# barbararoessle/e2e_multi_view_matching

Measured on AMD Instinct MI355X. Metric: image-pairs/sec @1024 kpts + pose AUC@5/10/20deg vs reference, higher is better.
Workload: dtype f16x2 (fp32 operands carried as 2 fp16 planes hi + 2^-11 lo', 22 significant bits, 3 fp16-MFMA products, fp32 accumulate; same 1e-4 / bit-exact-index parity bar); 1 GPU; configs[1]: tuple_size=2 (1 pair per tuple), 1024 keypoints, 256-dim f32 descriptors, GNN 9x1 = 18 layers, 100 Sinkhorn iters, batch 32 tuples/GPU = 32 pairs/GPU, w8pt pose per pair; pairs_per_gpu=32, global_pairs=32, weights=random init (timed), identity-like for the AUC leg, parallelism=tuple-sharded x1

## Files before the change

e2e_multi_view_matching_amd/csrc/attention_p2w.hip:

```cpp
#include <algorithm>
#include <type_traits>

#include "attention_p2.h"

namespace e2emv {

typedef __attribute__((ext_vector_type(16))) float aw_f32x16;

constexpr int AW_QT = 256;
constexpr int AW_TILEB = 64 * 256;
constexpr int AW_REGB = 2 * AW_TILEB;
constexpr int AW_ELS = 3 * AW_REGB;
constexpr int AW_QIMG = AW_ELS + 2048;
constexpr int AW_LDS = AW_QIMG + 3 * AW_TILEB;
constexpr int AW_PART_F = 68;
constexpr float AW_SINV = 1.f / P2_QS, AW_PLOG = 7.f, AW_LIMIT = 60000.f;

__device__ __forceinline__ void aw_wait_q_k0(p2_f16x8 (&q)[2][2][4]) {
    asm volatile("s_waitcnt vmcnt(0) lgkmcnt(0)\n\ts_barrier"
                 : "+a"(q[0][0][0]), "+a"(q[0][0][1]), "+a"(q[0][0][2]), "+a"(q[0][0][3]), "+a"(q[0][1][0]), "+a"(q[0][1][1]), "+a"(q[0][1][2]), "+a"(q[0][1][3]),
                   "+a"(q[1][0][0]), "+a"(q[1][0][1]), "+a"(q[1][0][2]), "+a"(q[1][0][3]), "+a"(q[1][1][0]), "+a"(q[1][1][1]), "+a"(q[1][1][2]), "+a"(q[1][1][3])
                 :: "memory");
}

template <int I, int N, class F>
__device__ __forceinline__ void aw_for(F&& f) {
    if constexpr (I < N) {
        f(std::integral_constant<int, I>{});
        aw_for<I + 1, N>(f);
    }
}

__device__ __forceinline__ unsigned aw_cvt_pk(float v0, float v1) {
    const p2_f32x2 vv = {v0, v1};
    return __builtin_bit_cast(unsigned, __builtin_convertvector(vv, p2_f16x2));
}
__device__ __forceinline__ float aw_fma(float a, float b, float c) {
    float d;
    asm volatile("v_fma_f32 %0, %1, %2, %3" : "=v"(d) : "v"(a), "v"(b), "v"(c));
    return d;
}
__device__ __forceinline__ float aw_exp2(float a) {
    float d;
    asm volatile("v_exp_f32 %0, %1" : "=v"(d) : "v"(a));
    return d;
}
__device__ __forceinline__ void aw_acc(float& sum, float a) { asm volatile("v_add_f32 %0, %0, %1" : "+v"(sum) : "v"(a)); }
__device__ __forceinline__ unsigned aw_cvt_pk_v(float v0, float v1) {
    unsigned d;
    asm volatile("v_cvt_pk_f16_f32 %0, %1, %2" : "=v"(d) : "v"(v0), "v"(v1));
    return d;
}
__device__ __forceinline__ unsigned aw_mixlo(unsigned hi, float v0) {
    unsigned lo;
    asm volatile("v_fma_mixlo_f16 %0, %1, -1.0, %2 op_sel_hi:[1,0,0]" : "=v"(lo) : "v"(hi), "v"(v0));
    return lo;
}
__device__ __forceinline__ unsigned aw_mixhi(unsigned lo, unsigned hi, float v1) {
    asm volatile("v_fma_mixhi_f16 %0, %1, -1.0, %2 op_sel:[1,0,0] op_sel_hi:[1,0,0]" : "+v"(lo) : "v"(hi), "v"(v1));
    return lo;
}
__device__ __forceinline__ unsigned aw_lo(unsigned hi, float v0, float v1) {
    unsigned lo;
    asm("v_fma_mixlo_f16 %0, %1, -1.0, %2 op_sel_hi:[1,0,0]\n\tv_fma_mixhi_f16 %0, %1, -1.0, %3 op_sel:[1,0,0] op_sel_hi:[1,0,0]"
        : "=&v"(lo) : "v"(hi), "v"(v0), "v"(v1));
    return lo;
}

__device__ __forceinline__ void aw_mfma_s(aw_f32x16& c, p2_f16x8 a, p2_f16x8 b) {
    asm volatile("v_mfma_f32_32x32x16_f16 %0, %1, %2, %0" : "+v"(c) : "v"(a), "a"(b));
}
__device__ __forceinline__ void aw_mfma_s0(aw_f32x16& c, p2_f16x8 a, p2_f16x8 b) {
    asm volatile("v_mfma_f32_32x32x16_f16 %0, %1, %2, 0" : "=&v"(c) : "v"(a), "a"(b));
}
__device__ __forceinline__ void aw_mfma_sa(aw_f32x16& c, p2_f16x8 a, p2_f16x8 b) {
    asm volatile("v_mfma_f32_32x32x16_f16 %0, %1, %2, %0" : "+v"(c) : "a"(a), "a"(b));
}
__device__ __forceinline__ void aw_mfma_sa0(aw_f32x16& c, p2_f16x8 a, p2_f16x8 b) {
    asm volatile("v_mfma_f32_32x32x16_f16 %0, %1, %2, 0" : "=&v"(c) : "a"(a), "a"(b));
}
__device__ __forceinline__ void aw_mfma_oa(aw_f32x16& c, p2_f16x8 a, p2_u32x4 b) {
    asm volatile("v_mfma_f32_32x32x16_f16 %0, %1, %2, %0" : "+a"(c) : "a"(a), "v"(b));
}
template <int IMM>
__device__ __forceinline__ void aw_read_frag(p2_f16x8& d, unsigned addr) {
    static_assert(IMM >= 0 && IMM < 65536, "ds_read offset: 16 bits");
    asm volatile("ds_read_b128 %0, %1 offset:%2" : "=a"(d) : "v"(addr), "n"(IMM));
}
template <int N>
__device__ __forceinline__ void aw_wait_frag(p2_f16x8 (&f)[4]) {
    asm volatile("s_waitcnt lgkmcnt(%4)" : "+a"(f[0]), "+a"(f[1]), "+a"(f[2]), "+a"(f[3]) : "n"(N));
}
template <bool HAS_E, bool MULTI = true, bool PART = false>
__global__ __launch_bounds__(256, 1) void attention_p2w_kernel(AttnP2Params p) {
    extern __shared__ __attribute__((aligned(16))) char smem_aw[];

    int lin = blockIdx.x, ks = 0;
    constexpr bool part = PART;
    if constexpr (PART) {
        const int h = blockIdx.x, tpx = (8 * p.gper * p.nq - p.n_full) >> 3;
        ks = (h >> 3) / tpx;
        lin = p.n_full + 8 * ((h >> 3) % tpx) + (h & 7);
    }
    const int xcd = lin & 7, idx = lin >> 3;
    const int g = xcd * p.gper + idx / p.nq;
    if (g >= p.groups) return;
    const int qt = idx % p.nq;
    const int img = g / p.H, head = g % p.H;
    const int b = img / p.T, t = img % p.T;
    if (qt * AW_QT >= p.nv[t]) return;

    const int tid = threadIdx.x, lane = tid & 63;
    const int wave = __builtin_amdgcn_readfirstlane(tid >> 6);
    const int l31 = lane & 31, lh = lane >> 5;
    const unsigned row_b = 8u * (unsigned)p.D;

    int q_row[2];
    bool q_ok[2];
    p2_f16x8 Qf[2][2][4];
#pragma unroll
    for (int a = 0; a < 2; ++a) {
        q_row[a] = qt * AW_QT + wave * 64 + a * 32 + l31;
        q_ok[a] = q_row[a] < p.n_rows;
    }
    const int q_blk = __builtin_amdgcn_readfirstlane(((int64_t)img * p.n_rows + min(qt * AW_QT + wave * 64, p.n_rows - 1)) >> 6);
    const int e_q_v = HAS_E ? p.EQK[q_blk * 8 + head] : 0;
    const unsigned q_img = wave == 0 ? 2u * AW_REGB : (unsigned)(AW_QIMG + (wave - 1) * AW_TILEB);
    {
        const __amdgpu_buffer_rsrc_t rsQ = __builtin_amdgcn_make_buffer_rsrc(const_cast<uint16_t*>(p.qk), 0, (int)p.qk_bytes, 0x00020000);
        const unsigned so = (unsigned)(img * p.n_rows) * row_b;
        asm volatile("" ::: "memory");
#pragma unroll
        for (int i = 0; i < 16; ++i) {
            const int rl = 4 * i + (lane >> 4);
            const int row = min(qt * AW_QT + wave * 64 + rl, p.n_rows - 1);
            const unsigned c = (unsigned)((lane & 15) ^ (rl & 15));
            p2_glds16(rsQ, smem_aw + q_img + i * 1024, (unsigned)row * row_b + (unsigned)head * 256u + c * 16u, so);
        }
        asm volatile("" ::: "memory");
    }
    const int e_q = __builtin_amdgcn_readfirstlane(e_q_v);

    const int n_src = p.cross ? p.T - 1 : 1;
    auto src_t = [&](int si) __attribute__((always_inline)) { return !p.cross ? t : (si < t ? si : si + 1); };
    int n_tiles = 0;
    for (int si = 0; si < n_src; ++si) n_tiles += (p.nv[src_t(si)] + 63) / 64;
    int t0 = 0;
    if constexpr (PART) {
        t0 = ks * n_tiles / p.n_split;
        n_tiles = (ks + 1) * n_tiles / p.n_split - t0;
        if (n_tiles <= 0) return;
    }
    struct Cur { int si, kt, nv; unsigned kb, vb; int eb; };
    auto cur_src = [&](Cur& c) __attribute__((always_inline)) {
        const int im = b * p.T + src_t(c.si);
        c.kt = 0;
        c.nv = p.nv[src_t(c.si)];
        c.kb = (unsigned)(im * p.n_rows) * row_b;
        c.vb = (unsigned)((im * p.H + head) * 64) * (unsigned)p.n_rows * 4u;
        c.eb = (im * p.n_rows) >> 6;
    };
    auto cur_next = [&](Cur& c) __attribute__((always_inline)) {
        ++c.kt;
        if constexpr (MULTI) {
            if (c.kt * 64 >= c.nv && c.si + 1 < n_src) { ++c.si; cur_src(c); }
        }
    };
    auto cur_init = [&]() __attribute__((always_inline)) {
        Cur c;
        c.si = 0;
        cur_src(c);
        if constexpr (PART)
            for (int i = 0; i < t0; ++i) cur_next(c);
        return c;
    };

    const __amdgpu_buffer_rsrc_t rsK = __builtin_amdgcn_make_buffer_rsrc(const_cast<uint16_t*>(p.qk), 0, (int)p.qk_bytes, 0x00020000);
    const __amdgpu_buffer_rsrc_t rsV = __builtin_amdgcn_make_buffer_rsrc(const_cast<uint16_t*>(p.vt), 0, (int)p.vt_bytes, 0x00020000);
    unsigned k_vo[4], v_vo[4];
#pragma unroll
    for (int i = 0; i < 4; ++i) {
        const int row = 4 * (wave * 4 + i) + (lane >> 4);
        const unsigned c = (unsigned)((lane & 15) ^ (row & 15));
        k_vo[i] = (unsigned)row * row_b + 4u * (unsigned)p.D + (unsigned)head * 256u + c * 16u;
        v_vo[i] = (unsigned)row * (unsigned)p.n_rows * 4u + c * 16u;
    }
    auto k_so = [&](const Cur& c) __attribute__((always_inline)) { return c.kb + (unsigned)c.kt * 64u * row_b; };
    auto v_so = [&](const Cur& c) __attribute__((always_inline)) { return c.vb + (unsigned)c.kt * 256u; };
    auto k_piece = [&](int region, int i, unsigned so) __attribute__((always_inline)) { p2_glds16(rsK, smem_aw + region * AW_REGB + AW_TILEB + (wave * 4 + i) * 1024, k_vo[i], so); };
    auto v_piece = [&](int region, int i, unsigned so) __attribute__((always_inline)) { p2_glds16(rsV, smem_aw + region * AW_REGB + (wave * 4 + i) * 1024, v_vo[i], so); };
    int* const els = reinterpret_cast<int*>(smem_aw + AW_ELS);
    int ek_mine = 0, ev_mine = 0;
    if (HAS_E && tid < n_tiles) {
        int si = 0, kt = PART ? tid + t0 : tid;
        if constexpr (MULTI) {
            for (; si + 1 < n_src; ++si) {
                const int nt = (p.nv[src_t(si)] + 63) / 64;
                if (kt < nt) break;
                kt -= nt;
            }
        }
        const int blk = (((b * p.T + src_t(si)) * p.n_rows) >> 6) + kt;
        ek_mine = p.EQK[blk * 8 + 4 + head];
        if (p.EVt) ev_mine = p.EVt[blk * 4 + head];
    }
    typedef __attribute__((address_space(3))) const p2_u32x2* lds_pair_t;
    const unsigned els0 = (unsigned)(uintptr_t)(__attribute__((address_space(3))) char*)smem_aw + (unsigned)AW_ELS;
    auto read_e = [&](int tl) __attribute__((always_inline)) {
        return *reinterpret_cast<lds_pair_t>((uintptr_t)(els0 + 8u * (unsigned)min(tl, n_tiles - 1)));
    };

    const int kz = l31 & 15;
    const unsigned lds0 = (unsigned)(uintptr_t)(__attribute__((address_space(3))) char*)smem_aw;
    unsigned R[4][2];
#pragma unroll
    for (int s = 0; s < 4; ++s)
#pragma unroll
        for (int pl = 0; pl < 2; ++pl)
            R[s][pl] = lds0 + (unsigned)(l31 * 256 + ((((s >> 1) * 8 + pl * 4 + 2 * (s & 1) + lh) ^ kz) << 4));
    typedef __attribute__((address_space(3))) const p2_f16x8* lds_frag_t;
    auto frag = [&](int s, int pl, int imm) __attribute__((always_inline)) { return *reinterpret_cast<lds_frag_t>((uintptr_t)(R[s][pl] + (unsigned)imm)); };

    constexpr int PA[3] = {1, 0, 0};
    constexpr int PB[3] = {0, 1, 0};

    aw_f32x16 O[2][2], S[2][2];
    p2_u32x4 Pf[2][2][4];
#pragma unroll
    for (int a = 0; a < 2; ++a)
#pragma unroll
        for (int d = 0; d < 2; ++d)
#pragma unroll
            for (int r = 0; r < 16; ++r) O[a][d][r] = 0.f;
    float m_run[2] = {-1e30f, -1e30f}, l_run[2] = {0.f, 0.f};
    int e_o = 0;
    bool o_started = false;
    unsigned n_slow = 0;

    auto sm_slow = [&](auto BB, float sinv, int valid) __attribute__((always_inline)) {
        constexpr int B = decltype(BB)::value;
        asm volatile("s_nop 15" : "+v"(S[B][0]), "+v"(S[B][1]), "+a"(O[B][0]), "+a"(O[B][1]));
        if (valid < 64) {
#pragma unroll
            for (int kb = 0; kb < 2; ++kb)
#pragma unroll
                for (int r = 0; r < 16; ++r)
                    if (kb * 32 + (r & 3) + 8 * (r >> 2) + 4 * lh >= valid) S[B][kb][r] = -INFINITY;
        }
        float mx = S[B][0][0];
#pragma unroll
        for (int kb = 0; kb < 2; ++kb)
#pragma unroll
            for (int r = 0; r < 16; ++r) mx = fmaxf(mx, S[B][kb][r]);
        {
            float x = mx, y = mx;
            asm volatile("s_nop 1\n\tv_permlane32_swap_b32 %0, %1\n\ts_nop 1" : "+v"(x), "+v"(y));
            mx = fmaxf(x, y);
        }
        mx *= sinv;
        const float m_new = fmaxf(m_run[B], mx);
        const float alpha = __builtin_amdgcn_exp2f(m_run[B] - m_new);
#pragma unroll
        for (int r = 0; r < 16; ++r) { O[B][0][r] *= alpha; O[B][1][r] *= alpha; }
        const float e0 = AW_PLOG - m_new;
        float ps = 0.f;
#pragma unroll
        for (int k = 0; k < 16; ++k) {
            const int kb = k >> 3, r = 2 * (k & 7), u = 2 * kb + ((k & 7) >> 2), e = k & 3;
            const float p0 = __builtin_amdgcn_exp2f(__builtin_fmaf(S[B][kb][r], sinv, e0));
            const float p1 = __builtin_amdgcn_exp2f(__builtin_fmaf(S[B][kb][r + 1], sinv, e0));
            ps += p0 + p1;
            const P2Pair pr = p2_split_plain(p0, p1);
            Pf[B][0][u][e] = pr.hi; Pf[B][1][u][e] = pr.lo;
        }
        l_run[B] = l_run[B] * alpha + ps;
        m_run[B] = m_new;
        asm volatile("s_nop 4" : "+a"(O[B][0]), "+a"(O[B][1]));
    };

    Cur cK = cur_init(), cV = cur_init(), cS = cur_init();
    int nK = 0, nV = 0;
    auto adv_k = [&]() __attribute__((always_inline)) { if (++nK < n_tiles) cur_next(cK); };
    auto adv_v = [&]() __attribute__((always_inline)) { if (++nV < n_tiles) cur_next(cV); };
    {
        const unsigned so = k_so(cK);
#pragma unroll
        for (int i = 0; i < 4; ++i) k_piece(2, i, so);
        adv_k();
    }
    unsigned so_v01[2], so_k12[2];
#pragma unroll
    for (int r = 0; r < 2; ++r) {
        so_v01[r] = v_so(cV);
        so_k12[r] = k_so(cK);
        adv_v();
        adv_k();
    }
    if (HAS_E && tid < n_tiles) { els[2 * tid] = ek_mine; els[2 * tid + 1] = ev_mine; }
#pragma unroll
    for (int s = 0; s < 4; ++s)
#pragma unroll
        for (int pl = 0; pl < 2; ++pl) R[s][pl] += q_img;
    asm volatile("s_waitcnt vmcnt(4)" ::: "memory");
    aw_for<0, 16>([&](auto II) __attribute__((always_inline)) {
        constexpr int a = decltype(II)::value >> 3, pl = (decltype(II)::value >> 2) & 1, s = decltype(II)::value & 3;
        aw_read_frag<a * 8192>(Qf[a][pl][s], R[s][pl]);
    });
    aw_wait_q_k0(Qf);
    p2_u32x2 e_pair = {0u, 0u};
    if constexpr (HAS_E) e_pair = read_e(0);
#pragma unroll
    for (int s = 0; s < 4; ++s)
#pragma unroll
        for (int pl = 0; pl < 2; ++pl) R[s][pl] += 2 * AW_REGB - q_img;
    {
        const float sinv = AW_SINV * p2_exp2i(e_q + __builtin_amdgcn_readfirstlane((int)e_pair[0]));
        p2_f16x8 kf[2][2][2];
#pragma unroll
        for (int kb = 0; kb < 2; ++kb)
#pragma unroll
            for (int pl = 0; pl < 2; ++pl) kf[0][kb][pl] = frag(0, pl, AW_TILEB + kb * 8192);
#pragma unroll
        for (int s = 0; s < 4; ++s) {
            if (s < 3) {
#pragma unroll
                for (int kb = 0; kb < 2; ++kb)
#pragma unroll
                    for (int pl = 0; pl < 2; ++pl) kf[(s + 1) & 1][kb][pl] = frag(s + 1, pl, AW_TILEB + kb * 8192);
            }
            __builtin_amdgcn_sched_barrier(0);
#pragma unroll
            for (int a = 0; a < 2; ++a)
#pragma unroll
                for (int q = 0; q < 3; ++q)
#pragma unroll
                    for (int kb = 0; kb < 2; ++kb) {
                        if (s == 0 && q == 0) aw_mfma_s0(S[a][kb], kf[s & 1][kb][PA[q]], Qf[a][PB[q]][s]);
                        else aw_mfma_s(S[a][kb], kf[s & 1][kb][PA[q]], Qf[a][PB[q]][s]);
                        const int slot = s * 12 + a * 6 + q * 2 + kb;
                        if (slot % 3 == 1) {
                            const int n = slot / 3, r = n >> 3, i = n & 3;
                            if ((n & 4) == 0) v_piece(r, i, so_v01[r]);
                            else k_piece(r, i, so_k12[r]);
                        }
                        __builtin_amdgcn_sched_barrier(0);
                    }
        }
        asm volatile("s_waitcnt vmcnt(8) lgkmcnt(0)\n\ts_barrier" ::: "memory");
        sm_slow(std::integral_constant<int, 0>{}, sinv, cS.nv - cS.kt * 64);
        if (cS.nv - cS.kt * 64 >= 64) {
            asm volatile("s_nop 15" : "+v"(S[1][0]), "+v"(S[1][1]));
            float mx = S[1][0][0];
#pragma unroll
            for (int kb = 0; kb < 2; ++kb)
#pragma unroll
                for (int r = 0; r < 16; ++r) mx = fmaxf(mx, S[1][kb][r]);
            float x = mx, y = mx;
            asm volatile("s_nop 1\n\tv_permlane32_swap_b32 %0, %1\n\ts_nop 1" : "+v"(x), "+v"(y));
            m_run[1] = fmaxf(x, y) * sinv;
        }
    }
#pragma unroll
    for (int s = 0; s < 4; ++s)
#pragma unroll
        for (int pl = 0; pl < 2; ++pl) R[s][pl] -= 2 * AW_REGB;
    int reg_cur = 0, seg_tile = 0;

    p2_f16x8 FA[8][4];
    auto read_frag = [&](auto GG, auto NN, auto SS, auto KK) __attribute__((always_inline)) {
        constexpr int G = decltype(GG)::value, N = decltype(NN)::value, S = decltype(SS)::value, KPART = decltype(KK)::value;
        constexpr int x = N & 1, pl = N < 2 ? 1 : 0;
        aw_read_frag<KPART * AW_TILEB + x * 8192>(FA[G][N], R[S][pl]);
    };
    aw_for<0, 8>([&](auto II) __attribute__((always_inline)) {
        constexpr int g = decltype(II)::value / 4, n = decltype(II)::value % 4;
        read_frag(std::integral_constant<int, g>{}, std::integral_constant<int, n>{}, std::integral_constant<int, g>{}, std::integral_constant<int, 0>{});
    });

    auto seg = [&](auto AA, auto LL) __attribute__((always_inline)) {
        constexpr int A = decltype(AA)::value, B = 1 - A;
        constexpr bool LAST = decltype(LL)::value;
        constexpr bool HAS_SM = !(LAST && A == 1);
        constexpr int NSLOT = LAST ? 24 : 48, NG = NSLOT / 6;
        constexpr int MPS = LAST ? 2 : 1;

        if (A == 0) {
            if (HAS_E && p.EVt) {
                const int e_v = __builtin_amdgcn_readfirstlane((int)e_pair[1]);
                if (__builtin_expect(o_started && e_v != e_o, 0)) {
                    const float f = e_o - e_v < -126 ? 0.f : p2_exp2i(e_o - e_v);
                    asm volatile("s_nop 15" : "+a"(O[0][0]), "+a"(O[0][1]), "+a"(O[1][0]), "+a"(O[1][1]));
#pragma unroll
                    for (int a = 0; a < 2; ++a)
#pragma unroll
                        for (int r = 0; r < 16; ++r) { O[a][0][r] *= f; O[a][1][r] *= f; }
                    asm volatile("s_nop 4" : "+a"(O[0][0]), "+a"(O[0][1]), "+a"(O[1][0]), "+a"(O[1][1]));
                }
                e_o = e_v;
                o_started = true;
            }
        }
        float sinv = AW_SINV, e0 = 0.f, ps = 0.f;
        int valid = 64;
        if (HAS_SM) {
            if (HAS_E) sinv = AW_SINV * p2_exp2i(e_q + __builtin_amdgcn_readfirstlane((int)e_pair[0]));
            if (HAS_E && A == 0 && !LAST) e_pair = read_e(seg_tile + 1);
            e0 = AW_PLOG - m_run[B];
            valid = cS.nv - cS.kt * 64;
        }
        if (HAS_SM && __builtin_expect(valid < 64, 0)) {
            asm volatile("s_nop 7" : "+v"(S[B][0]), "+v"(S[B][1]));
#pragma unroll
            for (int kb = 0; kb < 2; ++kb)
#pragma unroll
                for (int r = 0; r < 16; ++r)
                    if (kb * 32 + (r & 3) + 8 * (r >> 2) + 4 * lh >= valid) S[B][kb][r] = -INFINITY;
            asm volatile("" : "+v"(S[B][0]), "+v"(S[B][1]));
        }
        bool slow = false;
        float xa[16][2], pa[16][2], psA = 0.f, psB = 0.f, sinv_v = sinv;
        asm volatile("" : "+v"(sinv_v), "+v"(e0));
        unsigned hi_k[16], lo_k[16];
        auto micro = [&](auto MM) __attribute__((always_inline)) {
            constexpr int m = decltype(MM)::value;
            constexpr int k = m / 3, ph = m % 3;
            constexpr int kb = (k & 15) >> 3, r = 2 * (k & 7);
            if constexpr (m == 48) {
                lo_k[15] = aw_mixlo(hi_k[15], pa[15][0]);
            } else if constexpr (m == 49) {
                Pf[B][1][3][3] = aw_mixhi(lo_k[15], hi_k[15], pa[15][1]);
            } else if constexpr (ph == 0) {
                xa[k][0] = aw_fma(S[B][kb][r], sinv_v, e0);
                if constexpr (k > 0) lo_k[k - 1] = aw_mixlo(hi_k[k - 1], pa[k - 1][0]);
                xa[k][1] = aw_fma(S[B][kb][r + 1], sinv_v, e0);
            } else if constexpr (ph == 1) {
                pa[k][0] = aw_exp2(xa[k][0]);
                if constexpr (k > 0) {
                    constexpr int k1 = k - 1, u = 2 * (k1 >> 3) + ((k1 & 7) >> 2), e = k1 & 3;
                    Pf[B][1][u][e] = aw_mixhi(lo_k[k1], hi_k[k1], pa[k1][1]);
                }
                pa[k][1] = aw_exp2(xa[k][1]);
            } else {
                constexpr int u = 2 * (k >> 3) + ((k & 7) >> 2), e = k & 3;
                aw_acc(psA, pa[k][0]);
                hi_k[k] = aw_cvt_pk_v(pa[k][0], pa[k][1]);
                Pf[B][0][u][e] = hi_k[k];
                aw_acc(psB, pa[k][1]);
            }
        };

        unsigned so_v = 0, so_k = 0;
        if (A == 0 && !LAST) {
            so_v = v_so(cV);
            adv_v();
            so_k = k_so(cK);
            adv_k();
        }
        const int reg_ld = reg_cur == 0 ? 2 : reg_cur - 1;

        aw_for<0, NSLOT>([&](auto II) __attribute__((always_inline)) {
            constexpr int i = decltype(II)::value;
            constexpr int gq = i / 6, w = i % 6;
            if constexpr (A == 0 && w == 0) aw_wait_frag<(gq + 1 < NG ? 4 : 0)>(FA[gq]);
            if constexpr (i < 24) {
                constexpr int u = i / 6, q = (i % 6) / 2, db = i % 2;
                aw_mfma_oa(O[A][db], FA[u][db + 2 * (1 - PA[q])], Pf[A][PB[q]][u]);
            } else {
                constexpr int s = (i - 24) / 6, q = (i % 6) / 2, kb = i % 2;
                if constexpr (s == 0 && q == 0) aw_mfma_sa0(S[A][kb], FA[4 + s][kb + 2 * (1 - PA[q])], Qf[A][PB[q]][s]);
                else aw_mfma_sa(S[A][kb], FA[4 + s][kb + 2 * (1 - PA[q])], Qf[A][PB[q]][s]);
            }
            if constexpr (HAS_SM) {
                if constexpr (LAST) {
                    aw_for<0, MPS>([&](auto JJ) __attribute__((always_inline)) { micro(std::integral_constant<int, MPS * i + decltype(JJ)::value>{}); });
                } else if constexpr (i < 9) {
                    constexpr int m0 = i + i / 2 - (i > 0 && i % 2 == 0 ? 1 : 0);
                    micro(std::integral_constant<int, m0>{});
                    if constexpr (i >= 2 && i % 2 == 0) micro(std::integral_constant<int, m0 + 1>{});
                } else if constexpr (i < 46) {
                    micro(std::integral_constant<int, i + 4>{});
                } else if constexpr (i == 46) {
                    ps = psA;
                    aw_acc(ps, psB);
                } else if constexpr (i == 47) {
                    slow = __builtin_amdgcn_ballot_w64(!(ps < AW_LIMIT)) != 0;
                    l_run[B] += slow ? 0.f : ps;
                }
            }
            if constexpr (A == 1 && !LAST && i == 36) {
                asm volatile("s_waitcnt vmcnt(8) lgkmcnt(0)\n\ts_barrier" ::: "memory");
                const unsigned d = reg_cur == 2 ? (unsigned)(-2 * AW_REGB) : (unsigned)AW_REGB;
#pragma unroll
                for (int s = 0; s < 4; ++s)
#pragma unroll
                    for (int pl = 0; pl < 2; ++pl) R[s][pl] += d;
                reg_cur = reg_cur == 2 ? 0 : reg_cur + 1;
            }
            if constexpr (w >= 1 && w <= 4) {
                constexpr int gn = gq + 2;
                constexpr auto N = std::integral_constant<int, w - 1>{};
                if constexpr (A == 0 && gn < NG) {
                    if constexpr (gn < 4) read_frag(std::integral_constant<int, gn>{}, N, std::integral_constant<int, gn>{}, std::integral_constant<int, 0>{});
                    else read_frag(std::integral_constant<int, gn>{}, N, std::integral_constant<int, gn - 4>{}, std::integral_constant<int, 1>{});
                } else if constexpr (A == 1 && !LAST && gn >= NG) {
                    read_frag(std::integral_constant<int, gn - NG>{}, N, std::integral_constant<int, gn - NG>{}, std::integral_constant<int, 0>{});
                }
            }
            if constexpr (A == 0 && !LAST && i < 32 && i % 4 == 1) {
                if constexpr (i < 16) v_piece(reg_ld, i / 4, so_v);
                else k_piece(reg_ld, i / 4 - 4, so_k);
            }
            __builtin_amdgcn_sched_barrier(0);
        });

        if constexpr (HAS_SM && LAST) {
            lo_k[15] = aw_mixlo(hi_k[15], pa[15][0]);
            ps = psA + psB;
            Pf[B][1][3][3] = aw_mixhi(lo_k[15], hi_k[15], pa[15][1]);
            const bool slow = __builtin_amdgcn_ballot_w64(!(ps < AW_LIMIT)) != 0;
            l_run[B] += slow ? 0.f : ps;
            if (__builtin_expect(slow, 0)) {
                sm_slow(std::integral_constant<int, B>{}, sinv, valid);
                ++n_slow;
            }
        }
        if constexpr (HAS_SM && !LAST) {
            if (__builtin_expect(slow, 0)) {
                sm_slow(std::integral_constant<int, B>{}, sinv, valid);
                ++n_slow;
            }
        }
        if (A == 0) cur_next(cS);
    };

    for (int j = 0; j + 1 < n_tiles; ++j) {
        seg_tile = j;
        seg(std::integral_constant<int, 0>{}, std::false_type{});
        seg(std::integral_constant<int, 1>{}, std::false_type{});
    }
    seg(std::integral_constant<int, 0>{}, std::true_type{});
    seg(std::integral_constant<int, 1>{}, std::true_type{});

    asm volatile("s_waitcnt vmcnt(0)" ::: "memory");
    asm volatile("s_nop 15" : "+a"(O[0][0]), "+a"(O[0][1]), "+a"(O[1][0]), "+a"(O[1][1]));
    if constexpr (PART) {
        const int64_t rec = ((int64_t)(lin - p.n_full) * p.n_split + ks) * AW_QT;
        if (lane == 0) p.part_e[rec / 64 + wave] = e_o;
#pragma unroll
        for (int a = 0; a < 2; ++a) {
            const float l_tot = l_run[a] + __shfl_xor(l_run[a], 32);
            float* o = p.part + (rec + wave * 64 + a * 32 + l31) * AW_PART_F;
#pragma unroll
            for (int d = 0; d < 2; ++d)
#pragma unroll
                for (int gq = 0; gq < 4; ++gq)
                    *reinterpret_cast<p2_f32x4*>(o + 32 * d + 8 * gq + 4 * lh) = p2_f32x4{O[a][d][4 * gq], O[a][d][4 * gq + 1], O[a][d][4 * gq + 2], O[a][d][4 * gq + 3]};
            if (lh == 0) { o[64] = m_run[a]; o[65] = l_tot; }
        }
        if (p.stats && n_slow && lane == 0) atomicAdd(p.stats, n_slow);
        return;
    }
    if (p.EO && lane == 0 && q_ok[0]) p.EO[(((int64_t)img * p.n_rows + q_row[0]) >> 6) * 4 + head] = e_o;
#pragma unroll
    for (int a = 0; a < 2; ++a) {
        const float l_tot = l_run[a] + __shfl_xor(l_run[a], 32);
        const float inv = 1.f / (l_tot * P2_VS);
        uint16_t* op = p.out + p2_index((int64_t)img * p.n_rows + q_row[a], head * 64, p.D) + 8 * lh;
#pragma unroll
        for (int d = 0; d < 2; ++d)
#pragma unroll
            for (int kp = 0; kp < 2; ++kp) {
                const int r0 = 8 * kp, r1 = 8 * kp + 4;
                const P2Pair x0 = p2_split_scaled(O[a][d][r0] * inv, O[a][d][r0 + 1] * inv), x1 = p2_split_scaled(O[a][d][r0 + 2] * inv, O[a][d][r0 + 3] * inv);
                const P2Pair y0 = p2_split_scaled(O[a][d][r1] * inv, O[a][d][r1 + 1] * inv), y1 = p2_split_scaled(O[a][d][r1 + 2] * inv, O[a][d][r1 + 3] * inv);
                const auto h0 = __builtin_amdgcn_permlane32_swap(x0.hi, y0.hi, false, false), h1 = __builtin_amdgcn_permlane32_swap(x1.hi, y1.hi, false, false);
                const auto l0 = __builtin_amdgcn_permlane32_swap(x0.lo, y0.lo, false, false), l1 = __builtin_amdgcn_permlane32_swap(x1.lo, y1.lo, false, false);
                uint16_t* o = op + d * 64 + kp * 16;
                if (q_ok[a]) {
                    *reinterpret_cast<p2_u32x4*>(o) = p2_u32x4{h0[0], h1[0], h0[1], h1[1]};
                    *reinterpret_cast<p2_u32x4*>(o + 32) = p2_u32x4{l0[0], l1[0], l0[1], l1[1]};
                }
            }
    }
    if (p.stats && n_slow && lane == 0) atomicAdd(p.stats, n_slow);
}

__global__ __launch_bounds__(1024) void attention_p2w_combine(AttnP2Params p) {
    const int item = blockIdx.x, lin = p.n_full + item;
    const int xcd = lin & 7, idx = lin >> 3;
    const int g = xcd * p.gper + idx / p.nq;
    if (g >= p.groups) return;
    const int qt = idx % p.nq, img = g / p.H, head = g % p.H, t = img % p.T;
    if (qt * AW_QT >= p.nv[t]) return;
    const int n_src = p.cross ? p.T - 1 : 1;
    int n_tiles = 0;
    for (int si = 0; si < n_src; ++si) n_tiles += (p.nv[!p.cross ? t : (si < t ? si : si + 1)] + 63) / 64;
    const int q = threadIdx.x >> 2, dq = (threadIdx.x & 3) * 16;
    const int row = qt * AW_QT + q;
    float m = -3.0e38f;
    int e = -1000;
    for (int k = 0; k < p.n_split; ++k) {
// ... 90 lines not shown
```

Measured before the change: 3551 pairs/s.

## Hand-schedule attention MFMA groups with fused softmax and LDS reads in asm

Replaces the per-instruction asm wrappers and compiler-scheduled slot loop with large inline-asm groups. Each group interleaves six MFMAs with the exp/fma/cvt softmax micro-ops, ds_read fragment loads and waitcnt/barrier. Global-to-LDS loads now use immediate offsets off a shared LDS base, and the prologue S-MFMAs are grouped three per asm block. The aim is tighter control over instruction issue so that MFMA, VALU and LDS work overlap. The cost is fragile macro-generated asm whose register constraints could raise pressure or misorder dependencies.

Result: no change. 3544 pairs/s (-0.2%).

```diff
diff --git a/e2e_multi_view_matching_amd/csrc/attention_p2w.hip b/e2e_multi_view_matching_amd/csrc/attention_p2w.hip
--- a/e2e_multi_view_matching_amd/csrc/attention_p2w.hip
+++ b/e2e_multi_view_matching_amd/csrc/attention_p2w.hip
@@ -31,65 +31,183 @@
     }
 }
 
-__device__ __forceinline__ unsigned aw_cvt_pk(float v0, float v1) {
-    const p2_f32x2 vv = {v0, v1};
-    return __builtin_bit_cast(unsigned, __builtin_convertvector(vv, p2_f16x2));
-}
-__device__ __forceinline__ float aw_fma(float a, float b, float c) {
-    float d;
-    asm volatile("v_fma_f32 %0, %1, %2, %3" : "=v"(d) : "v"(a), "v"(b), "v"(c));
-    return d;
-}
-__device__ __forceinline__ float aw_exp2(float a) {
-    float d;
-    asm volatile("v_exp_f32 %0, %1" : "=v"(d) : "v"(a));
-    return d;
-}
-__device__ __forceinline__ void aw_acc(float& sum, float a) { asm volatile("v_add_f32 %0, %0, %1" : "+v"(sum) : "v"(a)); }
-__device__ __forceinline__ unsigned aw_cvt_pk_v(float v0, float v1) {
-    unsigned d;
-    asm volatile("v_cvt_pk_f16_f32 %0, %1, %2" : "=v"(d) : "v"(v0), "v"(v1));
-    return d;
-}
-__device__ __forceinline__ unsigned aw_mixlo(unsigned hi, float v0) {
-    unsigned lo;
-    asm volatile("v_fma_mixlo_f16 %0, %1, -1.0, %2 op_sel_hi:[1,0,0]" : "=v"(lo) : "v"(hi), "v"(v0));
-    return lo;
-}
-__device__ __forceinline__ unsigned aw_mixhi(unsigned lo, unsigned hi, float v1) {
-    asm volatile("v_fma_mixhi_f16 %0, %1, -1.0, %2 op_sel:[1,0,0] op_sel_hi:[1,0,0]" : "+v"(lo) : "v"(hi), "v"(v1));
-    return lo;
-}
-__device__ __forceinline__ unsigned aw_lo(unsigned hi, float v0, float v1) {
-    unsigned lo;
-    asm("v_fma_mixlo_f16 %0, %1, -1.0, %2 op_sel_hi:[1,0,0]\n\tv_fma_mixhi_f16 %0, %1, -1.0, %3 op_sel:[1,0,0] op_sel_hi:[1,0,0]"
-        : "=&v"(lo) : "v"(hi), "v"(v0), "v"(v1));
-    return lo;
-}
-
-__device__ __forceinline__ void aw_mfma_s(aw_f32x16& c, p2_f16x8 a, p2_f16x8 b) {
-    asm volatile("v_mfma_f32_32x32x16_f16 %0, %1, %2, %0" : "+v"(c) : "v"(a), "a"(b));
-}
-__device__ __forceinline__ void aw_mfma_s0(aw_f32x16& c, p2_f16x8 a, p2_f16x8 b) {
-    asm volatile("v_mfma_f32_32x32x16_f16 %0, %1, %2, 0" : "=&v"(c) : "v"(a), "a"(b));
-}
-__device__ __forceinline__ void aw_mfma_sa(aw_f32x16& c, p2_f16x8 a, p2_f16x8 b) {
-    asm volatile("v_mfma_f32_32x32x16_f16 %0, %1, %2, %0" : "+v"(c) : "a"(a), "a"(b));
-}
-__device__ __forceinline__ void aw_mfma_sa0(aw_f32x16& c, p2_f16x8 a, p2_f16x8 b) {
-    asm volatile("v_mfma_f32_32x32x16_f16 %0, %1, %2, 0" : "=&v"(c) : "a"(a), "a"(b));
-}
-__device__ __forceinline__ void aw_mfma_oa(aw_f32x16& c, p2_f16x8 a, p2_u32x4 b) {
-    asm volatile("v_mfma_f32_32x32x16_f16 %0, %1, %2, %0" : "+a"(c) : "a"(a), "v"(b));
-}
+#define AW_MFMA "v_mfma_f32_32x32x16_f16 "
+#define AW_MM(c, f, b) AW_MFMA "%[" #c "], %[" #f "], %[" #b "], %[" #c "]\n\t"
+#define AW_MZ(c, f, b) AW_MFMA "%[" #c "], %[" #f "], %[" #b "], 0\n\t"
+#define AW_TM0_OA AW_MM(c0, f0, bh)
+#define AW_TM1_OA AW_MM(c1, f1, bh)
+#define AW_TM2_OA AW_MM(c0, f2, bl)
+#define AW_TM3_OA AW_MM(c1, f3, bl)
+#define AW_TM4_OA AW_MM(c0, f2, bh)
+#define AW_TM5_OA AW_MM(c1, f3, bh)
+#define AW_O_OA [c0] "+a"(accO0), [c1] "+a"(accO1)
+#define AW_I_OA [bh] "v"(pbh), [bl] "v"(pbl)
+#define AW_TM0_SA AW_TM0_OA
+#define AW_TM1_SA AW_TM1_OA
+#define AW_TM2_SA AW_TM2_OA
+#define AW_TM3_SA AW_TM3_OA
+#define AW_TM4_SA AW_TM4_OA
+#define AW_TM5_SA AW_TM5_OA
+#define AW_O_SA [c0] "+v"(accS0), [c1] "+v"(accS1)
+#define AW_I_SA [bh] "a"(qbh), [bl] "a"(qbl)
+#define AW_TM0_SA0 AW_MZ(c0, f0, bh)
+#define AW_TM1_SA0 AW_MZ(c1, f1, bh)
+#define AW_TM2_SA0 AW_TM2_OA
+#define AW_TM3_SA0 AW_TM3_OA
+#define AW_TM4_SA0 AW_TM4_OA
+#define AW_TM5_SA0 AW_TM5_OA
+#define AW_O_SA0 [c0] "=&v"(accS0), [c1] "=&v"(accS1)
+#define AW_I_SA0 AW_I_SA
+#define AW_WAIT "s_waitcnt lgkmcnt(%[wn])\n\t"
+#define AW_O_HOMES [f0] "+a"(f0), [f1] "+a"(f1), [f2] "+a"(f2), [f3] "+a"(f3),
+#define AW_I_HOMES [f0] "a"(f0), [f1] "a"(f1), [f2] "a"(f2), [f3] "a"(f3),
+#define AW_O_READS [d0] "=&a"(d0), [d1] "=&a"(d1), [d2] "=&a"(d2), [d3] "=&a"(d3),
+#define AW_I_READS [r0] "v"(r0), [r1] "v"(r1), [i0] "n"(I0), [i1] "n"(I1),
+#define AW_RD(d, r, i) "ds_read_b128 %[" #d "], %[" #r "] offset:%[" #i "]\n\t"
+#define AW_TW_WR AW_WAIT
+#define AW_TB_WR ""
+#define AW_TR0_WR AW_RD(d0, r1, i0)
+#define AW_TR1_WR AW_RD(d1, r1, i1)
+#define AW_TR2_WR AW_RD(d2, r0, i0)
+#define AW_TR3_WR AW_RD(d3, r0, i1)
+#define AW_O_WR AW_O_HOMES AW_O_READS
+#define AW_I_WR [wn] "n"(WN), AW_I_READS
+#define AW_C_WR
+#define AW_TW_W AW_WAIT
+#define AW_TB_W ""
+#define AW_TR0_W ""
+#define AW_TR1_W ""
+#define AW_TR2_W ""
+#define AW_TR3_W ""
+#define AW_O_W AW_O_HOMES
+#define AW_I_W [wn] "n"(WN),
+#define AW_C_W
+#define AW_TW_N ""
+#define AW_TB_N ""
+#define AW_TR0_N ""
+#define AW_TR1_N ""
+#define AW_TR2_N ""
+#define AW_TR3_N ""
+#define AW_O_N
+#define AW_I_N AW_I_HOMES
+#define AW_C_N
+#define AW_TW_R ""
+#define AW_TB_R ""
+#define AW_TR0_R AW_TR0_WR
+#define AW_TR1_R AW_TR1_WR
+#define AW_TR2_R AW_TR2_WR
+#define AW_TR3_R AW_TR3_WR
+#define AW_O_R AW_O_READS
+#define AW_I_R AW_I_HOMES AW_I_READS
+#define AW_C_R
+#define AW_TW_RB ""
+#define AW_TB_RB "s_waitcnt vmcnt(8) lgkmcnt(0)\n\ts_barrier\n\t"
+#define AW_TR0_RB AW_TR0_WR
+#define AW_TR1_RB AW_TR1_WR
+#define AW_TR2_RB AW_TR2_WR
+#define AW_TR3_RB AW_TR3_WR
+#define AW_O_RB AW_O_READS
+#define AW_I_RB AW_I_R
+#define AW_C_RB "memory"
+#define AW_FMA(Z, h) "v_fma_f32 %[x" #Z #h "], %[s" #Z #h "], %[sv], %[e0]\n\t"
+#define AW_EXP(Z, h) "v_exp_f32 %[x" #Z #h "], %[x" #Z #h "]\n\t"
+#define AW_MIXLO(Y) "v_fma_mixlo_f16 %[l" #Y "], %[h" #Y "], -1.0, %[x" #Y "0] op_sel_hi:[1,0,0]\n\t"
+#define AW_MIXHI(Y) "v_fma_mixhi_f16 %[l" #Y "], %[h" #Y "], -1.0, %[x" #Y "1] op_sel:[1,0,0] op_sel_hi:[1,0,0]\n\t"
+#define AW_SUM(Z) "v_add_f32 %[za], %[za], %[x" #Z "0]\n\tv_cvt_pk_f16_f32 %[h" #Z "], %[x" #Z "0], %[x" #Z "1]\n\tv_add_f32 %[zb], %[zb], %[x" #Z "1]\n\t"
+#define AW_P0A(Z) AW_FMA(Z, 0) AW_FMA(Z, 1)
+#define AW_P1A(Z) AW_EXP(Z, 0) AW_EXP(Z, 1)
+#define AW_P0(Z, Y) AW_FMA(Z, 0) AW_MIXLO(Y) AW_FMA(Z, 1)
+#define AW_P1(Z, Y) AW_EXP(Z, 0) AW_MIXHI(Y) AW_EXP(Z, 1)
+#define AW_O_SUMS [za] "+v"(psA), [zb] "+v"(psB),
+#define AW_O_NEW(Z) [x##Z##0] "=&v"(x##Z##0), [x##Z##1] "=&v"(x##Z##1),
+#define AW_O_OLD(Z) [x##Z##0] "+v"(x##Z##0), [x##Z##1] "+v"(x##Z##1),
+#define AW_O_H(Z) [h##Z] "=&v"(h##Z),
+#define AW_O_L(Z) [l##Z] "=&v"(l##Z),
+#define AW_I_S(Z) [s##Z##0] "v"(s##Z##0), [s##Z##1] "v"(s##Z##1),
+#define AW_I_SCALE [sv] "v"(sinv_v), [e0] "v"(e0),
+#define AW_TS0_GN ""
+#define AW_TS1_GN ""
+#define AW_TS2_GN ""
+#define AW_TS3_GN ""
+#define AW_TS4_GN ""
+#define AW_TS5_GN ""
+#define AW_O_GN
+#define AW_I_GN
+#define AW_TS0_G0 AW_P0A(a)
+#define AW_TS1_G0 AW_P1A(a)
+#define AW_TS2_G0 AW_SUM(a) AW_P0(b, a)
+#define AW_TS3_G0 AW_P1(b, a)
+#define AW_TS4_G0 AW_SUM(b) AW_P0(c, b)
+#define AW_TS5_G0 AW_P1(c, b)
+#define AW_O_G0 AW_O_NEW(a) AW_O_H(a) AW_O_L(a) AW_O_NEW(b) AW_O_H(b) AW_O_L(b) AW_O_NEW(c) AW_O_SUMS
+#define AW_I_G0 AW_I_S(a) AW_I_S(b) AW_I_S(c) AW_I_SCALE
+#define AW_TS0_G1 AW_SUM(p) AW_P0(a, p)
+#define AW_TS1_G1 AW_P1(a, p)
+#define AW_TS2_G1 AW_SUM(a) AW_P0(b, a)
+#define AW_TS3_G1 AW_P1(b, a)
+#define AW_TS4_G1 AW_SUM(b)
+#define AW_TS5_G1 AW_P0(c, b)
+#define AW_O_G1 AW_O_H(p) AW_O_L(p) AW_O_NEW(a) AW_O_H(a) AW_O_L(a) AW_O_NEW(b) AW_O_H(b) AW_O_L(b) AW_O_NEW(c) AW_O_SUMS
+#define AW_I_G1 [xp0] "v"(xp0), [xp1] "v"(xp1), AW_I_S(a) AW_I_S(b) AW_I_S(c) AW_I_SCALE
+#define AW_TS0_GM AW_P1(a, p)
+#define AW_TS1_GM AW_SUM(a)
+#define AW_TS2_GM AW_P0(b, a)
+#define AW_TS3_GM AW_P1(b, a)
+#define AW_TS4_GM AW_SUM(b)
+#define AW_TS5_GM AW_P0(c, b)
+#define AW_O_GM AW_O_OLD(a) [lp] "+v"(lp), AW_O_H(a) AW_O_L(a) AW_O_NEW(b) AW_O_H(b) AW_O_L(b) AW_O_NEW(c) AW_O_SUMS
+#define AW_I_GM [hp] "v"(hp), [xp1] "v"(xp1), AW_I_S(b) AW_I_S(c) AW_I_SCALE
+#define AW_TS0_G7 AW_P1(a, p)
+#define AW_TS1_G7 AW_SUM(a)
+#define AW_TS2_G7 AW_MIXLO(a)
+#define AW_TS3_G7 AW_MIXHI(a)
+#define AW_TS4_G7 "v_add_f32 %[za], %[za], %[zb]\n\t"
+#define AW_TS5_G7 ""
+#define AW_O_G7 AW_O_OLD(a) [lp] "+v"(lp), AW_O_H(a) AW_O_L(a) AW_O_SUMS
+#define AW_I_G7 [hp] "v"(hp), [xp1] "v"(xp1),
+#define AW_TS0_L0 AW_P0A(a) AW_P1A(a)
+#define AW_TS1_L0 AW_SUM(a) AW_P0(b, a)
+#define AW_TS2_L0 AW_P1(b, a) AW_SUM(b)
+#define AW_TS3_L0 AW_P0(c, b) AW_P1(c, b)
+#define AW_TS4_L0 AW_SUM(c) AW_P0(d, c)
+#define AW_TS5_L0 AW_P1(d, c) AW_SUM(d)
+#define AW_O_L0 AW_O_NEW(a) AW_O_H(a) AW_O_L(a) AW_O_NEW(b) AW_O_H(b) AW_O_L(b) AW_O_NEW(c) AW_O_H(c) AW_O_L(c) AW_O_NEW(d) AW_O_H(d) AW_O_SUMS
+#define AW_I_L0 AW_I_S(a) AW_I_S(b) AW_I_S(c) AW_I_S(d) AW_I_SCALE
+#define AW_TS0_LM AW_P0(a, p) AW_P1(a, p)
+#define AW_TS1_LM AW_TS1_L0
+#define AW_TS2_LM AW_TS2_L0
+#define AW_TS3_LM AW_TS3_L0
+#define AW_TS4_LM AW_TS4_L0
+#define AW_TS5_LM AW_TS5_L0
+#define AW_O_LM AW_O_L(p) AW_O_L0
+#define AW_I_LM [hp] "v"(hp), [xp0] "v"(xp0), [xp1] "v"(xp1), AW_I_L0
+#define AW_GROUP_ASM(W, M, S)                                                \
+    asm volatile(AW_TW_##W                                                   \
+                 AW_TM0_##M AW_TS0_##S AW_TB_##W                             \
+                 AW_TM1_##M AW_TS1_##S AW_TR0_##W                            \
+                 AW_TM2_##M AW_TS2_##S AW_TR1_##W                            \
+                 AW_TM3_##M AW_TS3_##S AW_TR2_##W                            \
+                 AW_TM4_##M AW_TS4_##S AW_TR3_##W                            \
+                 AW_TM5_##M AW_TS5_##S                                       \
+                 : AW_O_##W AW_O_##S AW_O_##M : AW_I_##W AW_I_##S AW_I_##M : AW_C_##W)
+#define AW_GROUP_W(M, S)                                          \
+    if constexpr (WK == AW_WR) { AW_GROUP_ASM(WR, M, S); }        \
+    else if constexpr (WK == AW_W) { AW_GROUP_ASM(W, M, S); }     \
+    else if constexpr (WK == AW_N) { AW_GROUP_ASM(N, M, S); }     \
+    else if constexpr (WK == AW_R) { AW_GROUP_ASM(R, M, S); }     \
+    else { AW_GROUP_ASM(RB, M, S); }
+#define AW_GROUP_M(S)                                        \
+    if constexpr (MK == AW_OA) { AW_GROUP_W(OA, S) }         \
+    else if constexpr (MK == AW_SA) { AW_GROUP_W(SA, S) }    \
+    else { AW_GROUP_W(SA0, S) }
+enum { AW_OA, AW_SA, AW_SA0 };
+enum { AW_WR, AW_W, AW_N, AW_R, AW_RB };
+enum { AW_GN, AW_G0, AW_G1, AW_GM, AW_G7, AW_L0, AW_LM };
+
 template <int IMM>
 __device__ __forceinline__ void aw_read_frag(p2_f16x8& d, unsigned addr) {
     static_assert(IMM >= 0 && IMM < 65536, "ds_read offset: 16 bits");
     asm volatile("ds_read_b128 %0, %1 offset:%2" : "=a"(d) : "v"(addr), "n"(IMM));
-}
-template <int N>
-__device__ __forceinline__ void aw_wait_frag(p2_f16x8 (&f)[4]) {
-    asm volatile("s_waitcnt lgkmcnt(%4)" : "+a"(f[0]), "+a"(f[1]), "+a"(f[2]), "+a"(f[3]) : "n"(N));
 }
 template <bool HAS_E, bool MULTI = true, bool PART = false>
 __global__ __launch_bounds__(256, 1) void attention_p2w_kernel(AttnP2Params p) {
@@ -182,13 +300,23 @@
     for (int i = 0; i < 4; ++i) {
         const int row = 4 * (wave * 4 + i) + (lane >> 4);
         const unsigned c = (unsigned)((lane & 15) ^ (row & 15));
-        k_vo[i] = (unsigned)row * row_b + 4u * (unsigned)p.D + (unsigned)head * 256u + c * 16u;
-        v_vo[i] = (unsigned)row * (unsigned)p.n_rows * 4u + c * 16u;
+        k_vo[i] = (unsigned)row * row_b + 4u * (unsigned)p.D + (unsigned)head * 256u + c * 16u - 1024u * i;
+        v_vo[i] = (unsigned)row * (unsigned)p.n_rows * 4u + c * 16u - 1024u * i;
     }
     auto k_so = [&](const Cur& c) __attribute__((always_inline)) { return c.kb + (unsigned)c.kt * 64u * row_b; };
     auto v_so = [&](const Cur& c) __attribute__((always_inline)) { return c.vb + (unsigned)c.kt * 256u; };
-    auto k_piece = [&](int region, int i, unsigned so) __attribute__((always_inline)) { p2_glds16(rsK, smem_aw + region * AW_REGB + AW_TILEB + (wave * 4 + i) * 1024, k_vo[i], so); };
-    auto v_piece = [&](int region, int i, unsigned so) __attribute__((always_inline)) { p2_glds16(rsV, smem_aw + region * AW_REGB + (wave * 4 + i) * 1024, v_vo[i], so); };
+    auto piece = [&](const __amdgpu_buffer_rsrc_t rs, char* dst, int i, unsigned vo, unsigned so) __attribute__((always_inline)) {
+        typedef __attribute__((address_space(3))) void* lds_t;
+        const unsigned su = __builtin_amdgcn_readfirstlane(so);
+        switch (i) {
+            case 0: __builtin_amdgcn_raw_ptr_buffer_load_lds(rs, (lds_t)dst, 16, vo, su, 0, 0); break;
+            case 1: __builtin_amdgcn_raw_ptr_buffer_load_lds(rs, (lds_t)dst, 16, vo, su, 1024, 0); break;
+            case 2: __builtin_amdgcn_raw_ptr_buffer_load_lds(rs, (lds_t)dst, 16, vo, su, 2048, 0); break;
+            default: __builtin_amdgcn_raw_ptr_buffer_load_lds(rs, (lds_t)dst, 16, vo, su, 3072, 0); break;
+        }
+    };
+    auto k_piece = [&](int region, int i, unsigned so) __attribute__((always_inline)) { piece(rsK, smem_aw + region * AW_REGB + AW_TILEB + wave * 4096, i, k_vo[i], so); };
+    auto v_piece = [&](int region, int i, unsigned so) __attribute__((always_inline)) { piece(rsV, smem_aw + region * AW_REGB + wave * 4096, i, v_vo[i], so); };
     int* const els = reinterpret_cast<int*>(smem_aw + AW_ELS);
     int ek_mine = 0, ev_mine = 0;
     if (HAS_E && tid < n_tiles) {
@@ -221,8 +349,6 @@
     typedef __attribute__((address_space(3))) const p2_f16x8* lds_frag_t;
     auto frag = [&](int s, int pl, int imm) __attribute__((always_inline)) { return *reinterpret_cast<lds_frag_t>((uintptr_t)(R[s][pl] + (unsigned)imm)); };
 
-    constexpr int PA[3] = {1, 0, 0};
-    constexpr int PB[3] = {0, 1, 0};
 
     aw_f32x16 O[2][2], S[2][2];
     p2_u32x4 Pf[2][2][4];
@@ -332,19 +458,24 @@
 #pragma unroll
             for (int a = 0; a < 2; ++a)
 #pragma unroll
-                for (int q = 0; q < 3; ++q)
-#pragma unroll
-                    for (int kb = 0; kb < 2; ++kb) {
-                        if (s == 0 && q == 0) aw_mfma_s0(S[a][kb], kf[s & 1][kb][PA[q]], Qf[a][PB[q]][s]);
-                        else aw_mfma_s(S[a][kb], kf[s & 1][kb][PA[q]], Qf[a][PB[q]][s]);
-                        const int slot = s * 12 + a * 6 + q * 2 + kb;
-                        if (slot % 3 == 1) {
-                            const int n = slot / 3, r = n >> 3, i = n & 3;
-                            if ((n & 4) == 0) v_piece(r, i, so_v01[r]);
-                            else k_piece(r, i, so_k12[r]);
-                        }
-                        __builtin_amdgcn_sched_barrier(0);
-                    }
+                for (int hf = 0; hf < 2; ++hf) {
+                    aw_f32x16 &c0 = S[a][0], &c1 = S[a][1];
+                    const p2_f16x8 a0h = kf[s & 1][0][0], a0l = kf[s & 1][0][1], a1h = kf[s & 1][1][0], a1l = kf[s & 1][1][1];
+                    const p2_f16x8 bh = Qf[a][0][s], bl = Qf[a][1][s];
+                    if (hf == 0 && s == 0)
+                        asm volatile(AW_MZ(c0, a0l, bh) AW_MZ(c1, a1l, bh) AW_MM(c0, a0h, bl)
+                                     : [c0] "=&v"(c0), [c1] "=&v"(c1) : [a0l] "v"(a0l), [a1l] "v"(a1l), [a0h] "v"(a0h), [bh] "a"(bh), [bl] "a"(bl));
+                    else if (hf == 0)
+                        asm volatile(AW_MM(c0, a0l, bh) AW_MM(c1, a1l, bh) AW_MM(c0, a0h, bl)
+                                     : [c0] "+v"(c0), [c1] "+v"(c1) : [a0l] "v"(a0l), [a1l] "v"(a1l), [a0h] "v"(a0h), [bh] "a"(bh), [bl] "a"(bl));
+                    else
+                        asm volatile(AW_MM(c1, a1h, bl) AW_MM(c0, a0h, bh) AW_MM(c1, a1h, bh)
+                                     : [c0] "+v"(c0), [c1] "+v"(c1) : [a0h] "v"(a0h), [a1h] "v"(a1h), [bh] "a"(bh), [bl] "a"(bl));
+                    const int n = s * 4 + a * 2 + hf, r = n >> 3, i = n & 3;
+                    if ((n & 4) == 0) v_piece(r, i, so_v01[r]);
+                    else k_piece(r, i, so_k12[r]);
+                    __builtin_amdgcn_sched_barrier(0);
+                }
         }
         asm volatile("s_waitcnt vmcnt(8) lgkmcnt(0)\n\ts_barrier" ::: "memory");
         sm_slow(std::integral_constant<int, 0>{}, sinv, cS.nv - cS.kt * 64);
@@ -382,7 +513,6 @@
         constexpr bool LAST = decltype(LL)::value;
         constexpr bool HAS_SM = !(LAST && A == 1);
         constexpr int NSLOT = LAST ? 24 : 48, NG = NSLOT / 6;
-        constexpr int MPS = LAST ? 2 : 1;
 
         if (A == 0) {
             if (HAS_E && p.EVt) {
@@ -418,36 +548,9 @@
             asm volatile("" : "+v"(S[B][0]), "+v"(S[B][1]));
         }
         bool slow = false;
-        float xa[16][2], pa[16][2], psA = 0.f, psB = 0.f, sinv_v = sinv;
+        float xp[16][2], psA = 0.f, psB = 0.f, sinv_v = sinv;
         asm volatile("" : "+v"(sinv_v), "+v"(e0));
         unsigned hi_k[16], lo_k[16];
-        auto micro = [&](auto MM) __attribute__((always_inline)) {
-            constexpr int m = decltype(MM)::value;
-            constexpr int k = m / 3, ph = m % 3;
-            constexpr int kb = (k & 15) >> 3, r = 2 * (k & 7);
-            if constexpr (m == 48) {
-                lo_k[15] = aw_mixlo(hi_k[15], pa[15][0]);
-            } else if constexpr (m == 49) {
-                Pf[B][1][3][3] = aw_mixhi(lo_k[15], hi_k[15], pa[15][1]);
-            } else if constexpr (ph == 0) {
-                xa[k][0] = aw_fma(S[B][kb][r], sinv_v, e0);
-                if constexpr (k > 0) lo_k[k - 1] = aw_mixlo(hi_k[k - 1], pa[k - 1][0]);
-                xa[k][1] = aw_fma(S[B][kb][r + 1], sinv_v, e0);
-            } else if constexpr (ph == 1) {
-                pa[k][0] = aw_exp2(xa[k][0]);
-                if constexpr (k > 0) {
-                    constexpr int k1 = k - 1, u = 2 * (k1 >> 3) + ((k1 & 7) >> 2), e = k1 & 3;
-                    Pf[B][1][u][e] = aw_mixhi(lo_k[k1], hi_k[k1], pa[k1][1]);
-                }
-                pa[k][1] = aw_exp2(xa[k][1]);
-            } else {
-                constexpr int u = 2 * (k >> 3) + ((k & 7) >> 2), e = k & 3;
-                aw_acc(psA, pa[k][0]);
-                hi_k[k] = aw_cvt_pk_v(pa[k][0], pa[k][1]);
-                Pf[B][0][u][e] = hi_k[k];
-                aw_acc(psB, pa[k][1]);
-            }
-        };
 
         unsigned so_v = 0, so_k = 0;
         if (A == 0 && !LAST) {
@@ -458,37 +561,9 @@
         }
         const int reg_ld = reg_cur == 0 ? 2 : reg_cur - 1;
 
-        aw_for<0, NSLOT>([&](auto II) __attribute__((always_inline)) {
-            constexpr int i = decltype(II)::value;
-            constexpr int gq = i / 6, w = i % 6;
-            if constexpr (A == 0 && w == 0) aw_wait_frag<(gq + 1 < NG ? 4 : 0)>(FA[gq]);
-            if constexpr (i < 24) {
-                constexpr int u = i / 6, q = (i % 6) / 2, db = i % 2;
-                aw_mfma_oa(O[A][db], FA[u][db + 2 * (1 - PA[q])], Pf[A][PB[q]][u]);
-            } else {
-                constexpr int s = (i - 24) / 6, q = (i % 6) / 2, kb = i % 2;
-                if constexpr (s == 0 && q == 0) aw_mfma_sa0(S[A][kb], FA[4 + s][kb + 2 * (1 - PA[q])], Qf[A][PB[q]][s]);
-                else aw_mfma_sa(S[A][kb], FA[4 + s][kb + 2 * (1 - PA[q])], Qf[A][PB[q]][s]);
-            }
-            if constexpr (HAS_SM) {
-                if constexpr (LAST) {
-                    aw_for<0, MPS>([&](auto JJ) __attribute__((always_inline)) { micro(std::integral_constant<int, MPS * i + decltype(JJ)::value>{}); });
-                } else if constexpr (i < 9) {
-                    constexpr int m0 = i + i / 2 - (i > 0 && i % 2 == 0 ? 1 : 0);
-                    micro(std::integral_constant<int, m0>{});
-                    if constexpr (i >= 2 && i % 2 == 0) micro(std::integral_constant<int, m0 + 1>{});
-                } else if constexpr (i < 46) {
-                    micro(std::integral_constant<int, i + 4>{});
-                } else if constexpr (i == 46) {
-                    ps = psA;
-                    aw_acc(ps, psB);
-                } else if constexpr (i == 47) {
-                    slow = __builtin_amdgcn_ballot_w64(!(ps < AW_LIMIT)) != 0;
-                    l_run[B] += slow ? 0.f : ps;
-                }
-            }
-            if constexpr (A == 1 && !LAST && i == 36) {
-                asm volatile("s_waitcnt vmcnt(8) lgkmcnt(0)\n\ts_barrier" ::: "memory");
+        aw_for<0, NG>([&](auto GG) __attribute__((always_inline)) {
+            constexpr int g = decltype(GG)::value;
+            if constexpr (A == 1 && !LAST && g == 6) {
                 const unsigned d = reg_cur == 2 ? (unsigned)(-2 * AW_REGB) : (unsigned)AW_REGB;
 #pragma unroll
                 for (int s = 0; s < 4; ++s)
@@ -496,27 +571,69 @@
                     for (int pl = 0; pl < 2; ++pl) R[s][pl] += d;
                 reg_cur = reg_cur == 2 ? 0 : reg_cur + 1;
             }
-            if constexpr (w >= 1 && w <= 4) {
-                constexpr int gn = gq + 2;
-                constexpr auto N = std::integral_constant<int, w - 1>{};
-                if constexpr (A == 0 && gn < NG) {
-                    if constexpr (gn < 4) read_frag(std::integral_constant<int, gn>{}, N, std::integral_constant<int, gn>{}, std::integral_constant<int, 0>{});
-                    else read_frag(std::integral_constant<int, gn>{}, N, std::integral_constant<int, gn - 4>{}, std::integral_constant<int, 1>{});
-                } else if constexpr (A == 1 && !LAST && gn >= NG) {
-                    read_frag(std::integral_constant<int, gn - NG>{}, N, std::integral_constant<int, gn - NG>{}, std::integral_constant<int, 0>{});
+            constexpr int WN = g + 1 < NG ? 4 : 0;
+            [[maybe_unused]] p2_f16x8 &f0 = FA[g][0], &f1 = FA[g][1], &f2 = FA[g][2], &f3 = FA[g][3];
+            constexpr int MK = g < 4 ? AW_OA : (g == 4 ? AW_SA0 : AW_SA);
+            [[maybe_unused]] aw_f32x16 &accO0 = O[A][0], &accO1 = O[A][1], &accS0 = S[A][0], &accS1 = S[A][1];
+            [[maybe_unused]] const p2_u32x4 pbh = Pf[A][0][g & 3], pbl = Pf[A][1][g & 3];
+            [[maybe_unused]] const p2_f16x8 qbh = Qf[A][0][g & 3], qbl = Qf[A][1][g & 3];
+            constexpr int SK = !HAS_SM ? AW_GN : (LAST ? (g == 0 ? AW_L0 : AW_LM) : (g == 0 ? AW_G0 : (g == 1 ? AW_G1 : (g == 7 ? AW_G7 : AW_GM))));
+            constexpr int base = SK == AW_G1 ? 3 : (SK == AW_GM ? 2 * g + 1 : (SK == AW_G7 ? 15 : (LAST ? 4 * g : 0)));
+            constexpr int kp = (base + 15) & 15, ka = base & 15, kb = (base + 1) & 15, kc = (base + 2) & 15, kd = (base + 3) & 15;
+            [[maybe_unused]] const float sa0 = S[B][ka >> 3][2 * (ka & 7)], sa1 = S[B][ka >> 3][2 * (ka & 7) + 1], sb0 = S[B][kb >> 3][2 * (kb & 7)], sb1 = S[B][kb >> 3][2 * (kb & 7) + 1];
+            [[maybe_unused]] const float sc0 = S[B][kc >> 3][2 * (kc & 7)], sc1 = S[B][kc >> 3][2 * (kc & 7) + 1], sd0 = S[B][kd >> 3][2 * (kd & 7)], sd1 = S[B][kd >> 3][2 * (kd & 7) + 1];
+            [[maybe_unused]] float &xa0 = xp[ka][0], &xa1 = xp[ka][1], &xb0 = xp[kb][0], &xb1 = xp[kb][1], &xc0 = xp[kc][0], &xc1 = xp[kc][1], &xd0 = xp[kd][0], &xd1 = xp[kd][1];
+            [[maybe_unused]] const float xp0 = xp[kp][0], xp1 = xp[kp][1];
+            [[maybe_unused]] unsigned &hp = hi_k[kp], &ha = hi_k[ka], &hb = hi_k[kb], &hc = hi_k[kc], &hd = hi_k[kd];
+            [[maybe_unused]] unsigned &lp = lo_k[kp], &la = lo_k[ka], &lb = lo_k[kb], &lc = lo_k[kc];
+            constexpr bool RD = A == 0 ? g + 2 < NG : !LAST && g + 2 >= NG;
+            constexpr int G = RD ? (g + 2) % NG : 0;
+            constexpr int I0 = G >= 4 ? AW_TILEB : 0, I1 = I0 + 8192;
+            [[maybe_unused]] p2_f16x8 &d0 = FA[G][0], &d1 = FA[G][1], &d2 = FA[G][2], &d3 = FA[G][3];
+            [[maybe_unused]] const unsigned r0 = R[G & 3][0], r1 = R[G & 3][1];
+            constexpr int WK = A == 0 ? (RD ? AW_WR : AW_W) : (RD ? (g == 6 ? AW_RB : AW_R) : AW_N);
+            if constexpr (SK == AW_GN) { AW_GROUP_M(GN) }
+            else if constexpr (SK == AW_G0) { AW_GROUP_M(G0) }
+            else if constexpr (SK == AW_G1) { AW_GROUP_M(G1) }
+            else if constexpr (SK == AW_GM) { AW_GROUP_M(GM) }
+            else if constexpr (SK == AW_G7) { AW_GROUP_M(G7) }
+            else if constexpr (SK == AW_L0) { AW_GROUP_M(L0) }
+            else { AW_GROUP_M(LM) }
+            auto set_hi = [&](auto KK) __attribute__((always_inline)) { constexpr int k = decltype(KK)::value; Pf[B][0][2 * (k >> 3) + ((k & 7) >> 2)][k & 3] = hi_k[k]; };
+            auto set_lo = [&](auto KK) __attribute__((always_inline)) { constexpr int k = decltype(KK)::value; Pf[B][1][2 * (k >> 3) + ((k & 7) >> 2)][k & 3] = lo_k[k]; };
+            if constexpr (SK != AW_GN) {
+                set_hi(std::integral_constant<int, ka>{});
+                set_lo(std::integral_constant<int, ka>{});
+                if constexpr (SK == AW_G1) set_hi(std::integral_constant<int, kp>{});
+                if constexpr (SK != AW_G0 && SK != AW_L0) set_lo(std::integral_constant<int, kp>{});
+                if constexpr (SK != AW_G7) set_hi(std::integral_constant<int, kb>{});
+                if constexpr (SK == AW_G0 || SK == AW_L0 || SK == AW_LM) set_lo(std::integral_constant<int, kb>{});
+                if constexpr (SK == AW_L0 || SK == AW_LM) {
+                    set_hi(std::integral_constant<int, kc>{});
+                    set_lo(std::integral_constant<int, kc>{});
+                    set_hi(std::integral_constant<int, kd>{});
                 }
             }
-            if constexpr (A == 0 && !LAST && i < 32 && i % 4 == 1) {
-                if constexpr (i < 16) v_piece(reg_ld, i / 4, so_v);
-                else k_piece(reg_ld, i / 4 - 4, so_k);
+            if constexpr (SK == AW_G7) {
+                ps = psA;
+                slow = __builtin_amdgcn_ballot_w64(!(ps < AW_LIMIT)) != 0;
+                l_run[B] += slow ? 0.f : ps;
+            }
+            if constexpr (A == 0 && !LAST) {
+                if constexpr (g < 4) v_piece(reg_ld, g, so_v);
+                else k_piece(reg_ld, g - 4, so_k);
             }
             __builtin_amdgcn_sched_barrier(0);
         });
 
         if constexpr (HAS_SM && LAST) {
-            lo_k[15] = aw_mixlo(hi_k[15], pa[15][0]);
-            ps = psA + psB;
-            Pf[B][1][3][3] = aw_mixhi(lo_k[15], hi_k[15], pa[15][1]);
+            {
+                unsigned &la = lo_k[15], &ha = hi_k[15];
+                float &xa0 = xp[15][0], &xa1 = xp[15][1];
+                asm volatile(AW_MIXLO(a) "v_add_f32 %[ps], %[za], %[zb]\n\t" AW_MIXHI(a)
+                             : [la] "=&v"(la), [ps] "=&v"(ps) : [ha] "v"(ha), [xa0] "v"(xa0), [xa1] "v"(xa1), [za] "v"(psA), [zb] "v"(psB));
+                Pf[B][1][3][3] = la;
+            }
             const bool slow = __builtin_amdgcn_ballot_w64(!(ps < AW_LIMIT)) != 0;
             l_run[B] += slow ? 0.f : ps;
             if (__builtin_expect(slow, 0)) {
```
